# pxl-th/Monodepth2.jl

Hardware: NVIDIA B200
Metric: train frames/s @416x128 R18: view-synthesis loss path (warp + SSIM/L1 loss, fwd+bwd, 4 scales) (higher is better)
Workload: dtype f32

## Files before the change

monodepth2.jl_b200/csrc/md2_common.cuh:

```cuda
#pragma once
#include <cuda_runtime.h>
#include <stdint.h>
#include <string>
#include <stdio.h>

#include "../../include/md2.h"
#include "md2_math.cuh"

namespace md2 {

std::string& last_error_ref();
int set_error(const char* fmt, ...);

struct Workspace {
    void* ptr = nullptr;
    size_t bytes = 0;
};

}

enum { MD2_WS_PARTIAL = 0, MD2_WS_SUMS, MD2_WS_POSE, MD2_WS_STATS, MD2_WS_DISP, MD2_WS_GDISP,
       MD2_WS_MISC, MD2_WS_AUTOMASK, MD2_WS_COUNT };
enum { MD2_WS_BANKS = 1 + MD2_HOST_LANES };

#include <vector>
struct md2_ctx {
    int device;
    int64_t launches;
    int sm_count = 148;
    int bank = 0;
    int64_t ws_gen[MD2_WS_BANKS] = {};
    md2::Workspace ws[MD2_WS_BANKS][MD2_WS_COUNT];
    int prof_on = 0;
    std::vector<cudaEvent_t> prof_ev;
    size_t prof_used = 0;
    void* host[MD2_HOST_LANES] = {};
    void* opt = nullptr;
    void* taps = nullptr;
    void* replay = nullptr;
};

namespace md2 {

void* ws_get(md2_ctx* ctx, int slot, size_t bytes);
int launch_automask(md2_ctx* ctx, int S, const float* const* frames, const int64_t* frame_ns, const float* target, int64_t target_ns,
                    float* out, int W, int H, int C, int N, cudaStream_t st);

struct DeviceGuard {
    int prev = -1;
    cudaError_t err;
    explicit DeviceGuard(int device) {
        err = cudaGetDevice(&prev);
        if (err == cudaSuccess && prev != device) err = cudaSetDevice(device); else if (err == cudaSuccess) prev = -1;
// ... 74 lines not shown
```

monodepth2.jl_b200/csrc/md2_fused.cu:

```cuda
#include <stdarg.h>
#include <string.h>

#include <atomic>

#include "md2_common.cuh"
#include "md2_fused.cuh"
#include "md2_march.cuh"
#include "md2_march2.cuh"

namespace md2 {

void host_path_destroy(md2_ctx* ctx);
void opt_path_destroy(md2_ctx* ctx);
void replay_destroy(md2_ctx* ctx);
void taps_destroy(md2_ctx* ctx);

std::string& last_error_ref() {
    static thread_local std::string e;
    return e;
}
int set_error(const char* fmt, ...) {
    char buf[512];
    va_list ap;
    va_start(ap, fmt);
    vsnprintf(buf, sizeof(buf), fmt, ap);
    va_end(ap);
    last_error_ref() = buf;
    return 1;
}
void* ws_get(md2_ctx* ctx, int slot, size_t bytes) {
    Workspace& w = ctx->ws[ctx->bank][slot];
    if (w.bytes >= bytes && w.ptr) return w.ptr;
    if (w.ptr) {
        cudaDeviceSynchronize();
        cudaFree(w.ptr);
        w.ptr = nullptr; w.bytes = 0;
    }
    size_t want = bytes + bytes / 4 + 256;
    ctx->ws_gen[ctx->bank]++;
    cudaError_t e = cudaMalloc(&w.ptr, want);
    if (e != cudaSuccess) {
        set_error("workspace cudaMalloc(%zu) failed: %s", want, cudaGetErrorString(e));
        w.ptr = nullptr;
        return nullptr;
    }
    w.bytes = want;
    return w.ptr;
}

__global__ void upsample_kernel(const float* __restrict__ in, float* __restrict__ out, int w, int h,
                                int W, int H, int CN) {
    const long long i = (long long)blockIdx.x * blockDim.x + threadIdx.x;
    if (i >= (long long)W * H * CN) return;
    const int x = (int)(i % W), y = (int)((i / W) % H);
    const long long cn = i / ((long long)W * H);
    const float sx = up_scale(w, W), sy = up_scale(h, H);
    int x0, x1, y0, y1; float fx, fy;
    up_taps(x, w, W, x0, x1, fx);
    up_taps(y, h, H, y0, y1, fy);
    const float* b = in + cn * w * h;
    out[i] = bilerp(b[y0 * w + x0], b[y0 * w + x1], b[y1 * w + x0], b[y1 * w + x1], fx, fy);
}

__global__ void upsample_bwd_kernel(const float* __restrict__ gout, float* __restrict__ gin, int w,
                                    int h, int W, int H, int CN) {
// ... 95 lines not shown
        return;
    }
    const bool do_zero = zero_blocks > 0;
    zero_blocks = zero_blocks < 0 ? -zero_blocks : zero_blocks;
    const int zb = blockIdx.x - nblk - 1, s = zb / zero_blocks, sl = zb - s * zero_blocks;
    const int total = C * p.W * p.H;
    const int per = ((total + zero_blocks - 1) / zero_blocks + 3) & ~3;
    const int i0 = sl * per, i1 = min(i0 + per, total);
    {
        const float* src = p.src[s] + (long long)n * p.src_ns[s];
        for (int i = i0 + 32 * (int)threadIdx.x; i < i1; i += 32 * (int)blockDim.x)
            asm volatile("prefetch.global.L2 [%0];" ::"l"(src + i));
        if (threadIdx.x == 0 && i1 > i0) asm volatile("prefetch.global.L2 [%0];" ::"l"(src + (i1 - 1)));
    }
    if (!do_zero || !p.gsrc[s]) return;
    float* g = p.gsrc[s] + (long long)n * p.src_ns[s];
    if ((reinterpret_cast<uintptr_t>(g) & 15) == 0) {
        for (int i = i0 + 4 * (int)threadIdx.x; i + 3 < i1; i += 4 * (int)blockDim.x) *reinterpret_cast<float4*>(g + i) = make_float4(0.f, 0.f, 0.f, 0.f);
        for (int i = i0 + ((i1 - i0) & ~3) + (int)threadIdx.x; i < i1; i += blockDim.x) g[i] = 0.f;
    } else {
        for (int i = i0 + (int)threadIdx.x; i < i1; i += blockDim.x) g[i] = 0.f;
    }
}

template <int C, int LMAX>
__global__ void __launch_bounds__(32 * PREP_WARPS, 3) prep_kernel(const __grid_constant__ FusedParams p, int strips, int chunks,
                                                               int nblk, int do_stats, float* __restrict__ pose_ab,
                                                               float* __restrict__ part, int zero_blocks) {
    const int n = blockIdx.y;
    pdl_trigger();
    if (blockIdx.x == 0 || (int)blockIdx.x > nblk) { prep_pose_or_zero<C>(p, nblk, pose_ab, zero_blocks); return; }
    const int W = p.W, H = p.H, HW = W * H;
    __shared__ float red[PREP_WARPS][3 * LMAX];
    const int lane = threadIdx.x & 31, warp = threadIdx.x >> 5;
    const int w = (blockIdx.x - 1) * PREP_WARPS + warp;
    const bool active = w < strips * chunks;
    const int cy = w / strips, sx = w - cy * strips;
    const int gx = sx * PREP_COLS + lane;
    const int gxc = gx < W ? gx : W - 1;
    const bool own_col = active && lane < PREP_COLS && gx < W;
    const bool has_right = own_col && gx + 1 < W;
    const int Y0 = active ? cy * PREP_ROWS : 0;
    int yo[PREP_ROWS + 1];
#pragma unroll
    for (int r = 0; r <= PREP_ROWS; ++r) yo[r] = min(Y0 + r, H - 1) * W;

// ... 77 lines not shown
            float v0 = 0.f, v1 = 0.f, v2 = 0.f;
#pragma unroll
            for (int r = 0; r <= PREP_ROWS; ++r) {
                if (r < PREP_ROWS) {
                    const float dr = __shfl_down_sync(0xffffffffu, d[r], 1);
                    v0 = fmaf(fabsf(d[r] - dr), wx[r], v0);
                    v2 += (own_col && Y0 + r < H) ? d[r] : 0.f;
                }
                if (r > 0) v1 = fmaf(fabsf(d[r - 1] - d[r]), wy[r], v1);
            }
            v0 = warp_sum(v0); v1 = warp_sum(v1); v2 = warp_sum(v2);
            if (lane == 0) { red[warp][3 * l] = v0; red[warp][3 * l + 1] = v1; red[warp][3 * l + 2] = v2; }
        }
    }
    if (!do_stats) return;
    __syncthreads();
    if ((int)threadIdx.x < 3 * p.L) {
        float s = 0.f;
#pragma unroll
        for (int k = 0; k < PREP_WARPS; ++k) s += red[k][threadIdx.x];
        const int l = threadIdx.x / 3, k = threadIdx.x - 3 * l;
        part[(((long long)l * p.N + n) * nblk + (blockIdx.x - 1)) * 4 + k] = s;
    }
}

__device__ __forceinline__ float warp_reduce_16(float (&v)[16]) {
    const int lane = threadIdx.x & 31;
#pragma unroll
    for (int half = 8; half >= 1; half >>= 1) {
        const bool up = (lane & half) != 0;
#pragma unroll
        for (int i = 0; i < half; ++i) {
            const float send = up ? v[i] : v[i + half];
            const float keep = up ? v[i + half] : v[i];
            v[i] = keep + __shfl_xor_sync(0xffffffffu, send, half);
        }
    }
    return v[0] + __shfl_xor_sync(0xffffffffu, v[0], 16);
}

template <int C, int NLOW>
__global__ void __launch_bounds__(32 * PREP_WARPS, MD2_PREP_MINB) prep_fast_kernel(const __grid_constant__ FusedParams p, int strips, int chunks,
                                                                    int nblk, float* __restrict__ pose_ab,
                                                                    float* __restrict__ part, int zero_blocks) {
    constexpr int NS = NLOW + 1;
    static_assert(3 * NS <= 16, "one transpose-reduce of 16 values");
// ... 82 lines not shown
                if (r < PREP_ROWS && Y0 + r < H && own_col) out[yo[r]] = d[r];
            }
        }
#pragma unroll
        for (int r = 0; r <= PREP_ROWS; ++r) {
            if (r < PREP_ROWS) {
                const float dr = __shfl_down_sync(0xffffffffu, d[r], 1);
                v[3 * l] = fmaf(fabsf(d[r] - dr), wx[r], v[3 * l]);
                v[3 * l + 2] = fmaf(d[r], mcol * rowm[r], v[3 * l + 2]);
            }
            if (r > 0) v[3 * l + 1] = fmaf(fabsf(d[r - 1] - d[r]), wy[r], v[3 * l + 1]);
        }
    }
    const float tot = warp_reduce_16(v);
    if (lane < 16) red[warp][lane] = tot;
    __syncthreads();
    if ((int)threadIdx.x < 3 * NS) {
        float s = 0.f;
#pragma unroll
        for (int k = 0; k < PREP_WARPS; ++k) s += red[k][threadIdx.x];
        const int l = threadIdx.x / 3, k = threadIdx.x - 3 * l;
        part[(((long long)l * p.N + n) * nblk + (blockIdx.x - 1)) * 4 + k] = s;
    }
}

#ifndef MD2_ROLE_SWAP
#define MD2_ROLE_SWAP 1
#endif
template <int C, int S, bool BWD>
struct MarchCfg {
#ifndef MD2_MAXREG_C1
#define MD2_MAXREG_C1 128
#endif
#ifndef MD2_MAXREG_C3
#define MD2_MAXREG_C3 192
#endif
    static constexpr int MAXREG = C == 1 ? MD2_MAXREG_C1 : MD2_MAXREG_C3;
};

template <int C, int S, bool BWD>
__global__ void __maxnreg__((MarchCfg<C, S, BWD>::MAXREG))
march_kernel(const __grid_constant__ FusedParams p, int strips, int chunks, int q_full, int lgroups) {
    extern __shared__ __align__(16) float wsm[];
    using M = March<C, S, BWD>;
    constexpr int NP = M::NPART;
    const int lane = threadIdx.x & 31;
// ... 15 lines not shown
            asm volatile("mov.u32 %0, %%warpid;" : "=r"(wid));
            *swap_flag = MD2_ROLE_SWAP ? (int)((wid >> 2) & 1u) : 0;
        }
        __syncthreads();
        role ^= *swap_flag;
    }
    for (int it = blockIdx.x; it < items; it += gridDim.x) {
        const int z = it / ipi, rem = it - z * ipi;
        int cy, sx, sx_end;
        if (rem < n_full) { cy = rem / strips; sx = rem - cy * strips; sx_end = sx + 1; }
        else { cy = q_full; sx = (rem - n_full) * strips / lgroups; sx_end = (rem - n_full + 1) * strips / lgroups; }
        for (; sx < sx_end; ++sx) {
            float v[32];
            if (role == 0) M::run_forward(p, sx, cy, z, lane, wsm, gslot, v);
            else M::run_backward(p, sx, cy, z, lane, wsm, gslot, v);
            const float tot = warp_reduce_32(v);
            if (role == 0 ? lane < (BWD ? NSTAT : NP) : (lane >= NSTAT && lane < NP))
                p.partial[((long long)z * ipg + cy * strips + sx) * NP + lane] = tot;
            if (BWD) __syncthreads();
        }
    }
}

template <int C, int S, bool AM, bool DBG, bool GRAD>
__global__ void __maxnreg__((March2<C, S, AM, DBG, GRAD>::MAXREG))
march2_kernel(const __grid_constant__ FusedParams p, int strips, int chunks, int q_full, int lgroups) {
    extern __shared__ __align__(16) float wsm[];
    using M = March2<C, S, AM, DBG, GRAD>;
    constexpr int NP = M::NPART;
    const int lane = threadIdx.x;
    pdl_trigger();
    pdl_wait();
    const int ipg = strips * chunks;
    const int n_full = strips * q_full;
    const int ipi = n_full + (chunks > q_full ? lgroups : 0);
    const int items = ipi * p.L * p.N;
    for (int it = blockIdx.x; it < items; it += gridDim.x) {
        const int z = it / ipi, rem = it - z * ipi;
        int cy, sx, sx_end;
        if (rem < n_full) { cy = rem / strips; sx = rem - cy * strips; sx_end = sx + 1; }
        else { cy = q_full; sx = (rem - n_full) * strips / lgroups; sx_end = (rem - n_full + 1) * strips / lgroups; }
        for (; sx < sx_end; ++sx) {
            float v[32];
            M::run(p, sx, cy, z, lane, wsm, v);
            const float tot = warp_reduce_32(v);
            if (GRAD ? (lane == 0 || (lane >= NSTAT && lane < NP)) : lane < NSTAT)
                p.partial[((long long)z * ipg + cy * strips + sx) * NP + lane] = tot;
        }
    }
}

__device__ __forceinline__ double warp_sum_d(double v) {
#pragma unroll
    for (int o = 16; o > 0; o >>= 1) v += __shfl_xor_sync(0xffffffffu, v, o);
    return v;
}

constexpr int FIN_MAXROWS = 64;
constexpr int FIN_THREADS = 128;
#ifndef MD2_FIN_MINB
#define MD2_FIN_MINB 7
#endif
#ifndef MD2_FIN_UNROLL
#define MD2_FIN_UNROLL 16
#endif
constexpr int FIN_UNROLL = MD2_FIN_UNROLL;
#ifndef MD2_FIN_TIMING
#define MD2_FIN_TIMING 0
#endif

__global__ void __launch_bounds__(FIN_THREADS, MD2_FIN_MINB) finish_kernel(const __grid_constant__ FusedParams p, int NP, int ipg, int bwd, int low_rows) {
    extern __shared__ __align__(16) float vrow[];
    const int lane = threadIdx.x & 31, warp = threadIdx.x >> 5;
    pdl_wait();
    const int LN = p.L * p.N;
    int b = blockIdx.x;
    if (b == 0) {
        if (p.mode == 1 || MD2_FIN_TIMING == 4) return;
        constexpr int GL = 4;
        const int sub = threadIdx.x & (GL - 1);
        for (int z0 = 0; z0 < LN; z0 += FIN_THREADS / GL) {
            const int z = z0 + (threadIdx.x / GL);
            float v[4] = {0.f, 0.f, 0.f, 0.f};
            if (z < LN) {
                const float* pp = p.partial + (long long)z * ipg * NP;
                if (p.mode == 0) {
#pragma unroll 4
                    for (int it = sub; it < ipg; it += GL) {
#pragma unroll
                        for (int k = 0; k < 4; ++k) v[k] += __ldcg(pp + (long long)it * NP + k);
                    }
                } else {
#pragma unroll 8
                    for (int it = sub; it < ipg; it += GL) v[0] += __ldcg(pp + (long long)it * NP);
                    const float4* q = reinterpret_cast<const float4*>(p.prep_part) + (long long)z * p.prep_nblk;
#pragma unroll 8
                    for (int it = sub; it < p.prep_nblk; it += GL) {
                        const float4 t = __ldcg(q + it);
                        v[1] += t.x; v[2] += t.y; v[3] += t.z;
                    }
                }
            }
#pragma unroll
            for (int o = GL / 2; o > 0; o >>= 1)
#pragma unroll
                for (int k = 0; k < 4; ++k) v[k] += __shfl_xor_sync(0xffffffffu, v[k], o);
            if (z < LN && sub == 0) {
                float* st = p.stats_out + (long long)z * NSTAT;
#pragma unroll
                for (int k = 0; k < NSTAT; ++k) st[k] = v[k];
                if (p.saved && p.saved != p.stats_out)
#pragma unroll
                    for (int k = 0; k < NSTAT; ++k) p.saved[(long long)z * NSTAT + k] = v[k];
            }
        }
        __syncthreads();
        if (warp == 0 && p.loss) {
            const double P = (double)p.W * p.H;
            const double cx = 1.0 / ((double)(p.W - 1) * p.H * p.N), cy = 1.0 / ((double)p.W * (p.H - 1) * p.N);
            const double rPN = 1.0 / (P * p.N);
            double acc = 0.0;
            for (int z = lane; z < LN; z += 32) {
                const float* st = p.stats_out + (long long)z * NSTAT;
                const double m = p.normalize_disp ? ((double)st[3] / P + 1e-7) : 1.0;
                acc += (double)st[0] * rPN + (double)p.smooth_w[z / p.N] * (cx * st[1] + cy * st[2]) / m;
            }
            acc = warp_sum_d(acc);
            if (lane == 0) *p.loss = (float)(acc * p.loss_scale);
        }
        return;
    }
    b -= 1;
    if (!bwd) return;
    if (b < p.S * p.N) {
        if (MD2_FIN_TIMING == 2) return;
        constexpr int FIN_PR = FIN_THREADS / 3;
        __shared__ double pacc[FIN_PR][12];
        const int s = b / p.N, nn = b % p.N;
        const int q4 = threadIdx.x % 3, j = threadIdx.x / 3;
        if (j < FIN_PR) {
            double a0 = 0.0, a1 = 0.0, a2 = 0.0, a3 = 0.0;
            const int rows = p.L * ipg;
#pragma unroll 4
            for (int r = j; r < rows; r += FIN_PR) {
                const int l = r / ipg, it = r - l * ipg;
                const float4 t = __ldcg(reinterpret_cast<const float4*>(p.partial + (((long long)l * p.N + nn) * ipg + it) * NP + NSTAT + 12 * s) + q4);
                a0 += (double)t.x; a1 += (double)t.y; a2 += (double)t.z; a3 += (double)t.w;
            }
            pacc[j][4 * q4] = a0; pacc[j][4 * q4 + 1] = a1; pacc[j][4 * q4 + 2] = a2; pacc[j][4 * q4 + 3] = a3;
        }
        __syncthreads();
        if (threadIdx.x < 12) {
            double a = 0.0;
#pragma unroll 6
            for (int q = 0; q < FIN_PR; ++q) a += pacc[q][threadIdx.x];
            pacc[0][threadIdx.x] = a;
        }
        __syncthreads();
        if (threadIdx.x == 0 && MD2_FIN_TIMING != 1) finalize_pose(p.pose, s, nn, &pacc[0][0], &pacc[0][0] + 9);
        return;
    }
// ... 212 lines not shown
        if (rem) {
            if (rem < 8 && env <= 0) continue;
            int k = (int)((R + over) / (rem + over));
            if (k < 1) k = 1;
            if (k > strips) k = strips;
            lg = cdiv(strips, k);
            if (env_group >= 1) lg = env_group < strips ? env_group : strips;
        }
        const long long items = base * q + (rem ? (long long)LN * lg : 0);
        const double longest = rem ? fmax(R + over, cdiv(strips, lg) * (rem + over)) : R + over;
        const double total = (double)base * q * (R + over) + (rem ? (double)base * (rem + over) : 0.0);
        const long long per_sm = (items + sms - 1) / sms;
        const double thr = total / ((double)sms * warps);
        const double chain = (double)((per_sm + warps - 1) / warps) * longest;
        const double cost = thr > chain ? thr : chain;
        if (cost < best - 1e-9) { best = cost; best_R = R; group = lg; }
        if (R == 8) break;
    }
    return best_R;
}

struct TapsEntry {
    int W, H, L, dw[MAX_L], dh[MAX_L];
    int wcount[MAX_L] = {};
    float* dev = nullptr;
    uint64_t last_use = 0;
};
struct TapsCache {
    static constexpr int CAP = 8;
    TapsEntry e[CAP];
    int used = 0;
    uint64_t tick = 0;
};
void taps_destroy(md2_ctx* ctx) {
    TapsCache* tc = static_cast<TapsCache*>(ctx->taps);
    if (!tc) return;
    for (int i = 0; i < tc->used; ++i)
        if (tc->e[i].dev) cudaFree(tc->e[i].dev);
    delete tc;
    ctx->taps = nullptr;
}
static int taps_get(md2_ctx* ctx, const md2_vsl_desc* d, FusedParams& p, cudaStream_t st) {
    if (!ctx->taps) ctx->taps = new TapsCache();
    TapsCache* tc = static_cast<TapsCache*>(ctx->taps);
    ++tc->tick;
    TapsEntry* hit = nullptr;
    for (int i = 0; i < tc->used && !hit; ++i) {
        TapsEntry& e = tc->e[i];
        if (e.W == d->W && e.H == d->H && e.L == d->L && memcmp(e.dw, d->disp_w, sizeof(int) * d->L) == 0 && memcmp(e.dh, d->disp_h, sizeof(int) * d->L) == 0) hit = &e;
    }
    const int W = d->W, H = d->H;
    if (!hit) {
        cudaStreamCaptureStatus cs = cudaStreamCaptureStatusNone;
        if (cudaStreamIsCapturing(st, &cs) != cudaSuccess || cs != cudaStreamCaptureStatusNone)
            return set_error("internal: tap tables of a new shape requested under stream capture");
        if (tc->used < TapsCache::CAP) hit = &tc->e[tc->used++];
        else {
            hit = &tc->e[0];
            for (int i = 1; i < tc->used; ++i) if (tc->e[i].last_use < hit->last_use) hit = &tc->e[i];
            MD2_CHECK(cudaDeviceSynchronize());
            cudaFree(hit->dev); hit->dev = nullptr;
            for (int b = 0; b < MD2_WS_BANKS; ++b) ctx->ws_gen[b]++;
        }
        std::vector<float> h;
        for (int l = 0; l < d->L; ++l) {
            if (d->disp_w[l] == W && d->disp_h[l] == H) continue;
            std::vector<int> i0s[2], i1s[2];
            std::vector<float> fs[2];
            for (int pass = 0; pass < 2; ++pass) {
                const int n = pass ? H : W, m = pass ? d->disp_h[l] : d->disp_w[l];
                i0s[pass].resize(n); i1s[pass].resize(n); fs[pass].resize(n);
                for (int x = 0; x < n; ++x) {
                    up_taps(x, m, n, i0s[pass][x], i1s[pass][x], fs[pass][x]);
                    float e[4] = {0.f, 0.f, fs[pass][x], 0.f};
                    memcpy(&e[0], &i0s[pass][x], 4); memcpy(&e[1], &i1s[pass][x], 4);
                    h.insert(h.end(), e, e + 4);
                }
            }
            std::vector<float> wts;
            for (int pass = 0; pass < 2; ++pass) {
                const int n = pass ? H : W, m = pass ? d->disp_h[l] : d->disp_w[l];
                for (int i = 0; i < m; ++i) {
                    auto wgt = [&](int x) { return (i0s[pass][x] == i ? 1.f - fs[pass][x] : 0.f) + (i1s[pass][x] == i ? fs[pass][x] : 0.f); };
                    int lo = 0, hi = n - 1;
                    while (lo < hi && wgt(lo) == 0.f) ++lo;
                    while (hi > lo && wgt(hi) == 0.f) --hi;
                    const int cnt = hi - lo + 1, start = (int)wts.size();
                    for (int x = lo; x <= hi; ++x) wts.push_back(wgt(x));
                    float e[4] = {0.f, 0.f, 0.f, 0.f};
                    memcpy(&e[0], &lo, 4); memcpy(&e[1], &cnt, 4); memcpy(&e[2], &start, 4);
                    h.insert(h.end(), e, e + 4);
                }
            }
            while (wts.size() & 3) wts.push_back(0.f);
            h.insert(h.end(), wts.begin(), wts.end());
            hit->wcount[l] = (int)wts.size();
        }
        MD2_CHECK(cudaMalloc(&hit->dev, sizeof(float) * (h.size() + 4)));
        MD2_CHECK(cudaMemcpy(hit->dev, h.data(), sizeof(float) * h.size(), cudaMemcpyHostToDevice));
        hit->W = W; hit->H = H; hit->L = d->L;
        memset(hit->dw, 0, sizeof(hit->dw)); memset(hit->dh, 0, sizeof(hit->dh));
        memcpy(hit->dw, d->disp_w, sizeof(int) * d->L); memcpy(hit->dh, d->disp_h, sizeof(int) * d->L);
    }
    hit->last_use = tc->tick;
    const float* q = hit->dev;
    for (int l = 0; l < d->L; ++l) {
        if (d->disp_w[l] == W && d->disp_h[l] == H) { p.tap_x[l] = p.tap_y[l] = p.inv_x[l] = p.inv_y[l] = p.inv_w[l] = nullptr; continue; }
        p.tap_x[l] = q; q += (size_t)4 * W;
        p.tap_y[l] = q; q += (size_t)4 * H;
        p.inv_x[l] = q; q += (size_t)4 * d->disp_w[l];
        p.inv_y[l] = q; q += (size_t)4 * d->disp_h[l];
        p.inv_w[l] = q; q += (size_t)hit->wcount[l];
    }
    return 0;
}

static int check_desc(const md2_vsl_desc* d, bool need_loss_inputs) {
    MD2_REQUIRE(d != nullptr, "null descriptor");
    MD2_REQUIRE(d->W >= 2 && d->H >= 2 && d->W <= 65535 && d->H <= 32767, "W, H must be in 2..65535 / 2..32767");
    MD2_REQUIRE((long long)d->W * d->H * d->C < (1LL << 31), "one image must have fewer than 2^31 elements");
    MD2_REQUIRE(d->W <= 12288, "W must be <= 12288 (one image row is staged in shared memory)");
    MD2_REQUIRE(d->N >= 1, "N must be >= 1");
    MD2_REQUIRE(d->C == 1 || d->C == 3, "C must be 1 or 3");
    MD2_REQUIRE(d->S >= 1 && d->S <= MAX_S, "S must be 1 or 2");
    MD2_REQUIRE(d->K && d->invK, "K / invK are null");
    for (int s = 0; s < d->S; ++s) {
        MD2_REQUIRE(d->source[s] != nullptr, "null source image");
        MD2_REQUIRE(d->rot[s] && d->trans[s], "null pose");
    }
    if (need_loss_inputs) {
        MD2_REQUIRE(d->L >= 1 && d->L <= MAX_L, "L must be in 1..8");
        MD2_REQUIRE((long long)d->L * d->N <= 65535, "L*N too large");
        MD2_REQUIRE(d->target != nullptr, "null target image");
        for (int l = 0; l < d->L; ++l) {
            MD2_REQUIRE(d->disparity[l] != nullptr, "null disparity");
// ... 43 lines not shown
        int64_t ns[MAX_S];
        for (int s = 0; s < S; ++s) ns[s] = d->source_image_stride[s];
        if (launch_automask(ctx, S, d->source, ns, d->target, d->target_image_stride, am, W, H, C, N, st)) return 1;
        p.automask = am;
    }
    p.dbg = (bwd && !use_march_v1()) ? d->debug_choices : nullptr;
    if (d->debug_choices) MD2_REQUIRE(p.dbg != nullptr, "debug_choices is served by the value + gradient calls only");
    {
        const float mind = (float)(1.0 / (double)d->max_depth), maxd = (float)(1.0 / (double)d->min_depth);
        p.depth_a = maxd - mind; p.depth_b = mind;
    }
    int n_low = 0, low_rows = 0;
    for (int l = 0; l < L; ++l) {
        p.smooth_w[l] = d->smooth_weight[l];
        p.disp[l] = d->disparity[l]; p.dw[l] = d->disp_w[l]; p.dh[l] = d->disp_h[l];
        p.usx[l] = up_scale(d->disp_w[l], W); p.usy[l] = up_scale(d->disp_h[l], H);
        p.gdisp[l] = bwd ? d->grad_disparity[l] : nullptr;
        if (bwd) MD2_REQUIRE(d->grad_disparity[l] != nullptr, "null grad_disparity");
        if (d->disp_w[l] != W || d->disp_h[l] != H) {
            ++n_low;
            low_rows += d->disp_h[l];
        }
    }
    if (n_low && taps_get(ctx, d, p, st)) return 1;
    {
        const size_t img = (size_t)N * W * H;
        float* dscr = n_low ? (float*)ws_get(ctx, MD2_WS_DISP, sizeof(float) * img * n_low) : nullptr;
        float* gscr = (n_low && bwd) ? (float*)ws_get(ctx, MD2_WS_GDISP, sizeof(float) * img * n_low) : nullptr;
        if (n_low && (!dscr || (bwd && !gscr))) return 1;
        int k = 0;
        for (int l = 0; l < L; ++l) {
            const bool native = d->disp_w[l] == W && d->disp_h[l] == H;
            p.dfull[l] = native ? d->disparity[l] : dscr + img * k;
            p.gfull[l] = !bwd ? nullptr : (native ? d->grad_disparity[l] : gscr + img * k);
            if (!native) ++k;
        }
    }
    p.loss_scale = d->loss_scale;
    p.gloss = gloss;
    p.normalize_disp = d->normalize_disparity;
    p.mode = mode;
    fill_pose_io(d, p.pose);

    const bool v2 = !use_march_v1();
    p.m_R = choose_march_rows(W, H, L * N, v2 || bwd, ctx->sm_count, v2 ? march2_resident_of(C, S, p.automask != nullptr, bwd) : march_resident_of(C, S, bwd), p.m_group);
    static const bool dbg_env = getenv("MD2_DEBUG") != nullptr, generic_env = getenv("MD2_PREP_GENERIC") != nullptr;
    if (dbg_env) fprintf(stderr, "[md2] chunk height %d, %d groups of short last chunks per (scale, image)\n", p.m_R, p.m_group);
    const int tiles = cdiv(W, (v2 || bwd) ? 28 : 30) * cdiv(H, p.m_R);
    const int NP = NSTAT + 12 * S;
    p.pose_slot = 0;
    const int prep_strips = cdiv(W, PREP_COLS), prep_chunks = cdiv(H, PREP_ROWS);
    const int prep_nblk = cdiv((long long)prep_strips * prep_chunks, PREP_WARPS);
    const int do_stats = mode == MODE_FWDBWD;
    const bool zero_gs = bwd && d->zero_grad_source != 0;
    const int aux_blocks = bwd ? max(1, min(64, cdiv((long long)C * W * H, 8192))) : 0;
    const int zero_blocks = zero_gs ? aux_blocks : -aux_blocks;
    float* pose_ab = (float*)ws_get(ctx, MD2_WS_POSE, sizeof(float) * 24 * S * N);
    float* partial = (float*)ws_get(ctx, MD2_WS_PARTIAL, sizeof(float) * (size_t)tiles * L * N * NP);
    float* stats = (float*)ws_get(ctx, MD2_WS_STATS, sizeof(float) * (size_t)L * N * NSTAT);
    float* part2 = (float*)ws_get(ctx, MD2_WS_MISC, sizeof(float) * (size_t)prep_nblk * L * N * 4);
    if (!pose_ab || !partial || !stats || !part2) return 1;
    p.pose_ab = pose_ab; p.pose_e = pose_ab + (size_t)12 * S * N; p.partial = partial;
    p.stats = stats; p.stats_out = stats; p.saved = (mode == MODE_BWD) ? nullptr : d->saved;
    if (mode == MODE_BWD && d->saved) p.stats = d->saved;
    p.loss = (mode == MODE_BWD) ? nullptr : d->loss;
    p.prep_part = do_stats ? part2 : nullptr;
    p.prep_nblk = prep_nblk;

    cudaEvent_t evp0 = nullptr, evp3 = nullptr;
    if (ctx->prof_on == 2) {
        while (ctx->prof_used + 4 > ctx->prof_ev.size()) {
            cudaEvent_t e;
            MD2_CHECK(cudaEventCreate(&e));
            ctx->prof_ev.push_back(e);
        }
        evp0 = ctx->prof_ev[ctx->prof_used + 2]; evp3 = ctx->prof_ev[ctx->prof_used + 3];
        MD2_CHECK(cudaEventRecord(evp0, st));
    }
    {
        const int nb = (do_stats || n_low) ? prep_nblk : 0;
        dim3 g(1 + nb + S * aux_blocks, N);
        bool usual = nb > 0 && L >= 1 && L <= 4 && n_low == L - 1 && d->disp_w[L - 1] == W && d->disp_h[L - 1] == H;
        if (generic_env) usual = false;
#define MD2_PREPF(CC, NL) prep_fast_kernel<CC, NL><<<g, 32 * PREP_WARPS, 0, st>>>(p, prep_strips, prep_chunks, nb, pose_ab, part2, zero_blocks)
#define MD2_PREP(CC, LL) prep_kernel<CC, LL><<<g, 32 * PREP_WARPS, 0, st>>>(p, prep_strips, prep_chunks, nb, do_stats, pose_ab, part2, zero_blocks)
        if (usual && C == 1)      { if (L == 1) MD2_PREPF(1, 0); else if (L == 2) MD2_PREPF(1, 1); else if (L == 3) MD2_PREPF(1, 2); else MD2_PREPF(1, 3); }
        else if (usual)           { if (L == 1) MD2_PREPF(3, 0); else if (L == 2) MD2_PREPF(3, 1); else if (L == 3) MD2_PREPF(3, 2); else MD2_PREPF(3, 3); }
        else if (C == 1) { if (L == 1) MD2_PREP(1, 1); else if (L <= 4) MD2_PREP(1, 4); else MD2_PREP(1, 8); }
        else        { if (L == 1) MD2_PREP(3, 1); else if (L <= 4) MD2_PREP(3, 4); else MD2_PREP(3, 8); }
#undef MD2_PREPF
// ... 3 lines not shown

    cudaEvent_t ev0 = nullptr, ev1 = nullptr;
    if (ctx->prof_on) {
        if (ctx->prof_used + 2 > ctx->prof_ev.size()) {
            for (int k = 0; k < 2; ++k) {
                cudaEvent_t e;
                MD2_CHECK(cudaEventCreate(&e));
                ctx->prof_ev.push_back(e);
            }
        }
        ev0 = ctx->prof_ev[ctx->prof_used]; ev1 = ctx->prof_ev[ctx->prof_used + 1];
        ctx->prof_used += ctx->prof_on == 2 ? 4 : 2;
        MD2_CHECK(cudaEventRecord(ev0, st));
    }
    if (v2) {
        const bool viz = d->viz_loss || d->viz_warped[0] || (S > 1 && d->viz_warped[S - 1]);
        if (!bwd || viz) { if (dispatch_march2(ctx, C, S, p, st, false)) return 1; }
        if (bwd) { if (dispatch_march2(ctx, C, S, p, st, true)) return 1; }
    }
    else if (bwd) { if (dispatch_march<true>(ctx, C, S, p, st)) return 1; }
    else     { if (dispatch_march<false>(ctx, C, S, p, st)) return 1; }
    if (ev1) MD2_CHECK(cudaEventRecord(ev1, st));
    {
        const int blocks = 1 + (bwd ? S * N + low_rows * N : 0);
        MD2_CHECK(launch_after(2, finish_kernel, dim3(blocks), dim3(FIN_THREADS), sizeof(float) * ((W + 3) & ~3), st, p, NP, tiles, bwd ? 1 : 0, low_rows));
        MD2_LAUNCH_CHECK(ctx);
    }
    if (evp3) MD2_CHECK(cudaEventRecord(evp3, st));
    return 0;
}

struct ReplayEntry {
    md2_vsl_desc desc;
    int mode; float seed; int64_t ws_gen;
    uint64_t hash = 0;
    int seen = 0;
    cudaGraphExec_t exec = nullptr;
    int launches = 0;
    uint64_t last_use = 0;
};
struct ReplayCache {
    static constexpr int CAP = 64;
    ReplayEntry e[CAP];
    int used = 0;
    uint64_t tick = 0;
    cudaStream_t cap_stream = nullptr;
};
// ... 247 lines not shown
    return 0;
}

}

extern "C" {

const char* md2_version(void) { return "md2_b200 0.1.0 (sm_100a)"; }
const char* md2_last_error(void) { return md2::last_error_ref().c_str(); }

int md2_create(int device, md2_ctx** out) {
    if (!out) return md2::set_error("md2_create: null out pointer");
    int count = 0;
    cudaError_t e = cudaGetDeviceCount(&count);
    if (e != cudaSuccess || count == 0)
        return md2::set_error("md2_create: no CUDA device (%s); this library has no CPU fallback",
                              cudaGetErrorString(e));
    if (device < 0 || device >= count) return md2::set_error("md2_create: bad device %d", device);
    md2_ctx* c = new md2_ctx();
    c->device = device;
    c->launches = 0;
    c->sm_count = 148;
    cudaDeviceGetAttribute(&c->sm_count, cudaDevAttrMultiProcessorCount, device);
    *out = c;
    return 0;
}

int md2_destroy(md2_ctx* ctx) {
    if (!ctx) return 0;
    md2::DeviceGuard guard(ctx->device);
    cudaDeviceSynchronize();
    for (int b = 0; b < MD2_WS_BANKS; ++b)
        for (int i = 0; i < MD2_WS_COUNT; ++i)
            if (ctx->ws[b][i].ptr) cudaFree(ctx->ws[b][i].ptr);
    for (cudaEvent_t e : ctx->prof_ev) cudaEventDestroy(e);
    md2::host_path_destroy(ctx);
    md2::opt_path_destroy(ctx);
    md2::replay_destroy(ctx);
    md2::taps_destroy(ctx);
    delete ctx;
    return 0;
}

int64_t md2_launch_count(const md2_ctx* ctx) { return ctx ? ctx->launches : 0; }

int md2_profile_enable(md2_ctx* ctx, int32_t on) {
// ... 81 lines not shown
```

monodepth2.jl_b200/csrc/md2_fused.cuh:

```cuda
#pragma once
#include "md2_math.cuh"

namespace md2 {

constexpr int MAX_S = 2;
constexpr int MAX_L = 8;
constexpr int NSTAT = 4;

struct PoseIO {
    int mode;
    const float* rot[MAX_S];
    const float* trans[MAX_S];
    int invert[MAX_S];
    const float* K; const float* invK;
    float* grot[MAX_S];
    float* gtrans[MAX_S];
};

struct FusedParams {
    int W, H, N, L, S;
    const float* tgt; long long tgt_ns;
    const float* src[MAX_S]; long long src_ns[MAX_S];
    float* gsrc[MAX_S];
    const float* disp[MAX_L];
// ... 5 lines not shown
    const float* stats;
    float* partial;
    float depth_a, depth_b;
    float smooth_w[MAX_L];
    float loss_scale;
    float gloss;
    int normalize_disp;
    float* viz_warped[MAX_S];
    float* viz_loss;
    int mode;
    float* stats_out;
    float* saved;
    float* loss;
    PoseIO pose;
    int m_R, m_group, pose_slot;
    const float* dfull[MAX_L];
    float* gfull[MAX_L];
    const float* prep_part;
    int prep_nblk;
    float usx[MAX_L], usy[MAX_L];
    const float* tap_x[MAX_L]; const float* tap_y[MAX_L];
    const float* inv_x[MAX_L]; const float* inv_y[MAX_L]; const float* inv_w[MAX_L];
    int* dbg;
};

#if defined(__CUDA_ARCH__)
#define MD2_ATOMIC_ADD(p, v) atomicAdd((p), (v))
__device__ __forceinline__ float md2_rcp_approx(float x) {
    float r;
    asm("rcp.approx.ftz.f32 %0, %1;" : "=f"(r) : "f"(x));
    return r;
}
#define MD2_RCP_FAST(x) md2_rcp_approx(x)
#define MD2_EXP(x) __expf(x)
#else
#define MD2_ATOMIC_ADD(p, v) (*(p) += (v))
#define MD2_RCP_FAST(x) (1.0f / (x))
#define MD2_EXP(x) expf(x)
#endif

MD2_HD float rcp_acc(float x) {
#if defined(__CUDA_ARCH__)
    const float r = md2_rcp_approx(x);
    return fmaf(r, fmaf(-x, r, 1.0f), r);
#else
    return 1.0f / x;
// ... 184 lines not shown
```

Measured before the change: 106,700.

## Fuse tail reductions and disparity adjoint into prep and march kernels via last-block counters

```diff
diff --git a/monodepth2.jl_b200/csrc/md2_common.cuh b/monodepth2.jl_b200/csrc/md2_common.cuh
--- a/monodepth2.jl_b200/csrc/md2_common.cuh
+++ b/monodepth2.jl_b200/csrc/md2_common.cuh
@@ -20,7 +20,7 @@
 }
 
 enum { MD2_WS_PARTIAL = 0, MD2_WS_SUMS, MD2_WS_POSE, MD2_WS_STATS, MD2_WS_DISP, MD2_WS_GDISP,
-       MD2_WS_MISC, MD2_WS_AUTOMASK, MD2_WS_COUNT };
+       MD2_WS_MISC, MD2_WS_AUTOMASK, MD2_WS_COUNTERS, MD2_WS_GTOT, MD2_WS_COUNT };
 enum { MD2_WS_BANKS = 1 + MD2_HOST_LANES };
 
 #include <vector>
@@ -29,6 +29,7 @@
     int64_t launches;
     int sm_count = 148;
     int bank = 0;
+    int fin_legacy = 0;
     int64_t ws_gen[MD2_WS_BANKS] = {};
     md2::Workspace ws[MD2_WS_BANKS][MD2_WS_COUNT];
     int prof_on = 0;
diff --git a/monodepth2.jl_b200/csrc/md2_fused.cu b/monodepth2.jl_b200/csrc/md2_fused.cu
--- a/monodepth2.jl_b200/csrc/md2_fused.cu
+++ b/monodepth2.jl_b200/csrc/md2_fused.cu
@@ -1,6 +1,7 @@
 #include <stdarg.h>
 #include <string.h>
 
+#include <algorithm>
 #include <atomic>
 
 #include "md2_common.cuh"
@@ -41,6 +42,12 @@
     cudaError_t e = cudaMalloc(&w.ptr, want);
     if (e != cudaSuccess) {
         set_error("workspace cudaMalloc(%zu) failed: %s", want, cudaGetErrorString(e));
+        w.ptr = nullptr;
+        return nullptr;
+    }
+    if (slot == MD2_WS_COUNTERS && (e = cudaMemset(w.ptr, 0, want)) != cudaSuccess) {
+        set_error("workspace cudaMemset failed: %s", cudaGetErrorString(e));
+        cudaFree(w.ptr);
         w.ptr = nullptr;
         return nullptr;
     }
@@ -182,6 +189,36 @@
         for (int i = i0 + (int)threadIdx.x; i < i1; i += blockDim.x) g[i] = 0.f;
     }
 }
+
+__device__ __forceinline__ void prep_finish_image(const FusedParams& p, int nblk, const float* __restrict__ part, int L) {
+    __shared__ int last;
+    const int n = blockIdx.y;
+    __threadfence();
+    __syncthreads();
+    if (threadIdx.x == 0) {
+        last = atomicAdd(p.prep_cnt + n, 1) == nblk - 1;
+        if (last) p.prep_cnt[n] = 0;
+    }
+    __syncthreads();
+    const int lane = threadIdx.x & 31, l = threadIdx.x >> 5;
+    if (!last || l >= L) return;
+    __threadfence();
+    const float4* pp = reinterpret_cast<const float4*>(part) + ((long long)l * p.N + n) * nblk;
+    float a = 0.f, b = 0.f, c = 0.f;
+    for (int k = lane; k < nblk; k += 32) {
+        const float4 q = __ldcg(pp + k);
+        a += q.x; b += q.y; c += q.z;
+    }
+#pragma unroll
+    for (int o = 16; o > 0; o >>= 1) {
+        a += __shfl_xor_sync(0xffffffffu, a, o); b += __shfl_xor_sync(0xffffffffu, b, o); c += __shfl_xor_sync(0xffffffffu, c, o);
+    }
+    if (lane == 0) {
+        float* st = const_cast<float*>(p.stats) + ((long long)l * p.N + n) * NSTAT;
+        st[1] = a; st[2] = b; st[3] = c;
+    }
+}
+static_assert(MAX_L <= PREP_WARPS, "one warp per scale in prep_finish_image");
 
 template <int C, int LMAX>
 __global__ void __launch_bounds__(32 * PREP_WARPS, 3) prep_kernel(const __grid_constant__ FusedParams p, int strips, int chunks,
@@ -305,6 +342,7 @@
         const int l = threadIdx.x / 3, k = threadIdx.x - 3 * l;
         part[(((long long)l * p.N + n) * nblk + (blockIdx.x - 1)) * 4 + k] = s;
     }
+    if (p.prep_cnt) prep_finish_image(p, nblk, part, p.L);
 }
 
 __device__ __forceinline__ float warp_reduce_16(float (&v)[16]) {
@@ -433,6 +471,7 @@
         const int l = threadIdx.x / 3, k = threadIdx.x - 3 * l;
         part[(((long long)l * p.N + n) * nblk + (blockIdx.x - 1)) * 4 + k] = s;
     }
+    if (p.prep_cnt) prep_finish_image(p, nblk, part, NS);
 }
 
 #ifndef MD2_ROLE_SWAP
@@ -494,6 +533,114 @@
     }
 }
 
+template <int NP>
+__device__ __forceinline__ void march2_group_sum(const FusedParams& p, int z, int ipg, int lane) {
+    static_assert(NP % 4 == 0 && NP / 4 <= 8, "one float4 column per lane of a row set");
+    const int q = lane & 7, rs = lane >> 3;
+    double a[4] = {0.0, 0.0, 0.0, 0.0};
+    if (q < NP / 4) {
+        const float4* base = reinterpret_cast<const float4*>(p.partial + (long long)z * ipg * NP) + q;
+#pragma unroll 8
+        for (int r = rs; r < ipg; r += 4) {
+            const float4 t = __ldcg(base + (long long)r * (NP / 4));
+            a[0] += (double)t.x; a[1] += (double)t.y; a[2] += (double)t.z; a[3] += (double)t.w;
+        }
+    }
+#pragma unroll
+    for (int k = 0; k < 4; ++k) {
+        const double t0 = __shfl_sync(0xffffffffu, a[k], q), t1 = __shfl_sync(0xffffffffu, a[k], q + 8);
+        const double t2 = __shfl_sync(0xffffffffu, a[k], q + 16), t3 = __shfl_sync(0xffffffffu, a[k], q + 24);
+        a[k] = ((t0 + t1) + t2) + t3;
+    }
+    if (lane < NP / 4)
+#pragma unroll
+        for (int k = 0; k < 4; ++k) p.gtot[(long long)z * NP + 4 * lane + k] = a[k];
+}
+
+template <int SMEM>
+__device__ __forceinline__ void march2_adjoint_code(const FusedParams& p, int l, int n, int cx, int cc, int strips, int lane, float* wsm) {
+    const int* rng = p.adj_rng[l];
+    const int xa = rng[cx], xb = rng[cx + 1], ya = rng[2 * strips + cc], yb = rng[2 * strips + cc + 1];
+    if (xa >= xb || ya >= yb) return;
+    const float4* ix = reinterpret_cast<const float4*>(p.inv_x[l]);
+    const float4* iy = reinterpret_cast<const float4*>(p.inv_y[l]);
+    const float* __restrict__ wts = p.inv_w[l];
+    const int X0 = __float_as_int(__ldg(ix + xa).x);
+    const float4 el = __ldg(ix + xb - 1);
+    const int ncols = __float_as_int(el.x) + __float_as_int(el.y) - X0;
+    const int W = p.W, w = p.dw[l], h = p.dh[l], nxi = xb - xa;
+    const float* g = p.gfull[l] + (long long)n * W * p.H + X0;
+    float* gd = p.gdisp[l] + (long long)n * h * w;
+    const int rows_per = SMEM / ncols;
+    for (int y0 = ya; y0 < yb; y0 += rows_per) {
+        const int nyi = min(rows_per, yb - y0);
+        for (int j = lane; j < nyi * ncols; j += 32) {
+            const int r = j / ncols, c = j - r * ncols;
+            const float4 e = __ldg(iy + y0 + r);
+            const int ylo = __float_as_int(e.x), ny = __float_as_int(e.y);
+            const float* __restrict__ wy = wts + __float_as_int(e.z);
+            const float* gp = g + (long long)ylo * W + c;
+            float acc = 0.f;
+#pragma unroll 8
+            for (int k = 0; k < ny; ++k) acc = fmaf(__ldg(wy + k), __ldcg(gp + (long long)k * W), acc);
+            wsm[j] = acc;
+        }
+        __syncwarp();
+        for (int j = lane; j < nyi * nxi; j += 32) {
+            const int r = j / nxi, xi = xa + (j - r * nxi);
+            const float4 e = __ldg(ix + xi);
+            const int nx = __float_as_int(e.y);
+            const float* vr = wsm + r * ncols + (__float_as_int(e.x) - X0);
+            const float* __restrict__ wx = wts + __float_as_int(e.z);
+            float acc = 0.f;
+#pragma unroll 4
+            for (int k = 0; k < nx; ++k) acc = fmaf(__ldg(wx + k), vr[k], acc);
+            gd[(long long)(y0 + r) * w + xi] = acc;
+        }
+        __syncwarp();
+    }
+}
+
+__device__ __forceinline__ int march2_segment_count(const FusedParams& p, int sx, int cy, int z, int strips, int chunks, int lane) {
+    const int l = z / p.N, n = z - l * p.N;
+    int* acnt = p.adj_cnt[l];
+    __threadfence();
+    __syncwarp();
+    bool mine = false;
+    if (acnt) {
+        const int ncx = 2 * strips - 1, ncc = 2 * chunks - 1;
+        const int cx = 2 * sx + lane % 3 - 1, cc = 2 * cy + lane / 3 - 1;
+        if (lane < 9 && cx >= 0 && cx < ncx && cc >= 0 && cc < ncc) {
+            const int need = (1 + (cx & 1)) * (1 + (cc & 1));
+            if (need == 1) mine = true;
+            else {
+                int* c = acnt + ((long long)n * ncc + cc) * ncx + cx;
+                if (atomicAdd(c, 1) == need - 1) { *c = 0; mine = true; }
+            }
+        }
+    }
+    if (lane == 9) {
+        mine = atomicAdd(p.grp_cnt + z, 1) == strips * chunks - 1;
+        if (mine) p.grp_cnt[z] = 0;
+    }
+    return (int)__ballot_sync(0xffffffffu, mine);
+}
+
+template <int NP, int SMEM>
+__device__ __forceinline__ void march2_segment_finish(const FusedParams& p, int sx, int cy, int z, int strips, int chunks, int todo,
+                                                      int lane, float* wsm) {
+    const int l = z / p.N, n = z - l * p.N;
+    __threadfence();
+    if (todo & (1 << 9)) march2_group_sum<NP>(p, z, strips * chunks, lane);
+    todo &= (1 << 9) - 1;
+    while (todo) {
+        const int b = __ffs(todo) - 1;
+        todo &= todo - 1;
+        march2_adjoint_code<SMEM>(p, l, n, 2 * sx + b % 3 - 1, 2 * cy + b / 3 - 1, strips, lane, wsm);
+    }
+}
+constexpr int M2_PENDING = 8;
+
 template <int C, int S, bool AM, bool DBG, bool GRAD>
 __global__ void __maxnreg__((March2<C, S, AM, DBG, GRAD>::MAXREG))
 march2_kernel(const __grid_constant__ FusedParams p, int strips, int chunks, int q_full, int lgroups) {
@@ -507,6 +654,8 @@
     const int n_full = strips * q_full;
     const int ipi = n_full + (chunks > q_full ? lgroups : 0);
     const int items = ipi * p.L * p.N;
+    __shared__ int pend[GRAD ? M2_PENDING : 1][3];
+    int npend = 0;
     for (int it = blockIdx.x; it < items; it += gridDim.x) {
         const int z = it / ipi, rem = it - z * ipi;
         int cy, sx, sx_end;
@@ -518,7 +667,19 @@
             const float tot = warp_reduce_32(v);
             if (GRAD ? (lane == 0 || (lane >= NSTAT && lane < NP)) : lane < NSTAT)
                 p.partial[((long long)z * ipg + cy * strips + sx) * NP + lane] = tot;
-        }
+            if (GRAD && p.grp_cnt) {
+                const int todo = march2_segment_count(p, sx, cy, z, strips, chunks, lane);
+                if (todo && npend < M2_PENDING) {
+                    if (lane == 0) { pend[npend][0] = z; pend[npend][1] = sx | cy << 16; pend[npend][2] = todo; }
+                    ++npend;
+                }
+            }
+        }
+    }
+    for (int k = 0; k < npend; ++k) {
+        __syncwarp();
+        const int sc = pend[k][1];
+        march2_segment_finish<NP, M::SMEM_FLOATS>(p, sc & 0xffff, sc >> 16, pend[k][0], strips, chunks, pend[k][2], lane, wsm);
     }
 }
 
@@ -549,41 +710,54 @@
     int b = blockIdx.x;
     if (b == 0) {
         if (p.mode == 1 || MD2_FIN_TIMING == 4) return;
-        constexpr int GL = 4;
-        const int sub = threadIdx.x & (GL - 1);
-        for (int z0 = 0; z0 < LN; z0 += FIN_THREADS / GL) {
-            const int z = z0 + (threadIdx.x / GL);
-            float v[4] = {0.f, 0.f, 0.f, 0.f};
-            if (z < LN) {
-                const float* pp = p.partial + (long long)z * ipg * NP;
-                if (p.mode == 0) {
+        if (p.gtot) {
+            for (int z = threadIdx.x; z < LN; z += FIN_THREADS) {
+                const float* s3 = p.stats + (long long)z * NSTAT;
+                const float v[NSTAT] = {(float)__ldcg(p.gtot + (long long)z * NP), __ldcg(s3 + 1), __ldcg(s3 + 2), __ldcg(s3 + 3)};
+                float* st = p.stats_out + (long long)z * NSTAT;
+#pragma unroll
+                for (int k = 0; k < NSTAT; ++k) st[k] = v[k];
+                if (p.saved && p.saved != p.stats_out)
+#pragma unroll
+                    for (int k = 0; k < NSTAT; ++k) p.saved[(long long)z * NSTAT + k] = v[k];
+            }
+        } else {
+            constexpr int GL = 4;
+            const int sub = threadIdx.x & (GL - 1);
+            for (int z0 = 0; z0 < LN; z0 += FIN_THREADS / GL) {
+                const int z = z0 + (threadIdx.x / GL);
+                float v[4] = {0.f, 0.f, 0.f, 0.f};
+                if (z < LN) {
+                    const float* pp = p.partial + (long long)z * ipg * NP;
+                    if (p.mode == 0) {
 #pragma unroll 4
-                    for (int it = sub; it < ipg; it += GL) {
-#pragma unroll
-                        for (int k = 0; k < 4; ++k) v[k] += __ldcg(pp + (long long)it * NP + k);
-                    }
-                } else {
+                        for (int it = sub; it < ipg; it += GL) {
+#pragma unroll
+                            for (int k = 0; k < 4; ++k) v[k] += __ldcg(pp + (long long)it * NP + k);
+                        }
+                    } else {
 #pragma unroll 8
-                    for (int it = sub; it < ipg; it += GL) v[0] += __ldcg(pp + (long long)it * NP);
-                    const float4* q = reinterpret_cast<const float4*>(p.prep_part) + (long long)z * p.prep_nblk;
+                        for (int it = sub; it < ipg; it += GL) v[0] += __ldcg(pp + (long long)it * NP);
+                        const float4* q = reinterpret_cast<const float4*>(p.prep_part) + (long long)z * p.prep_nblk;
 #pragma unroll 8
-                    for (int it = sub; it < p.prep_nblk; it += GL) {
-                        const float4 t = __ldcg(q + it);
-                        v[1] += t.x; v[2] += t.y; v[3] += t.z;
+                        for (int it = sub; it < p.prep_nblk; it += GL) {
+                            const float4 t = __ldcg(q + it);
+                            v[1] += t.x; v[2] += t.y; v[3] += t.z;
+                        }
                     }
                 }
-            }
-#pragma unroll
-            for (int o = GL / 2; o > 0; o >>= 1)
-#pragma unroll
-                for (int k = 0; k < 4; ++k) v[k] += __shfl_xor_sync(0xffffffffu, v[k], o);
-            if (z < LN && sub == 0) {
-                float* st = p.stats_out + (long long)z * NSTAT;
-#pragma unroll
-                for (int k = 0; k < NSTAT; ++k) st[k] = v[k];
-                if (p.saved && p.saved != p.stats_out)
-#pragma unroll
-                    for (int k = 0; k < NSTAT; ++k) p.saved[(long long)z * NSTAT + k] = v[k];
+#pragma unroll
+                for (int o = GL / 2; o > 0; o >>= 1)
+#pragma unroll
+                    for (int k = 0; k < 4; ++k) v[k] += __shfl_xor_sync(0xffffffffu, v[k], o);
+                if (z < LN && sub == 0) {
+                    float* st = p.stats_out + (long long)z * NSTAT;
+#pragma unroll
+                    for (int k = 0; k < NSTAT; ++k) st[k] = v[k];
+                    if (p.saved && p.saved != p.stats_out)
+#pragma unroll
+                        for (int k = 0; k < NSTAT; ++k) p.saved[(long long)z * NSTAT + k] = v[k];
+                }
             }
         }
         __syncthreads();
@@ -609,6 +783,16 @@
         constexpr int FIN_PR = FIN_THREADS / 3;
         __shared__ double pacc[FIN_PR][12];
         const int s = b / p.N, nn = b % p.N;
+        if (p.gtot) {
+            if (threadIdx.x < 12) {
+                double a = 0.0;
+                for (int l = 0; l < p.L; ++l) a += __ldcg(p.gtot + ((long long)l * p.N + nn) * NP + NSTAT + 12 * s + threadIdx.x);
+                pacc[0][threadIdx.x] = a;
+            }
+            __syncthreads();
+            if (threadIdx.x == 0 && MD2_FIN_TIMING != 1) finalize_pose(p.pose, s, nn, &pacc[0][0], &pacc[0][0] + 9);
+            return;
+        }
         const int q4 = threadIdx.x % 3, j = threadIdx.x / 3;
         if (j < FIN_PR) {
             double a0 = 0.0, a1 = 0.0, a2 = 0.0, a3 = 0.0;
@@ -867,7 +1051,10 @@
 
 struct TapsEntry {
     int W, H, L, dw[MAX_L], dh[MAX_L];
+    int R;
     int wcount[MAX_L] = {};
+    int roff[MAX_L] = {};
+    bool adj_ok = false;
     float* dev = nullptr;
     uint64_t last_use = 0;
 };
@@ -885,14 +1072,15 @@
     delete tc;
     ctx->taps = nullptr;
 }
-static int taps_get(md2_ctx* ctx, const md2_vsl_desc* d, FusedParams& p, cudaStream_t st) {
+constexpr int M2_OW = 28;
+static int taps_get(md2_ctx* ctx, const md2_vsl_desc* d, FusedParams& p, cudaStream_t st, int R, bool& adj_ok) {
     if (!ctx->taps) ctx->taps = new TapsCache();
     TapsCache* tc = static_cast<TapsCache*>(ctx->taps);
     ++tc->tick;
     TapsEntry* hit = nullptr;
     for (int i = 0; i < tc->used && !hit; ++i) {
         TapsEntry& e = tc->e[i];
-        if (e.W == d->W && e.H == d->H && e.L == d->L && memcmp(e.dw, d->disp_w, sizeof(int) * d->L) == 0 && memcmp(e.dh, d->disp_h, sizeof(int) * d->L) == 0) hit = &e;
+        if (e.W == d->W && e.H == d->H && e.L == d->L && e.R == R && memcmp(e.dw, d->disp_w, sizeof(int) * d->L) == 0 && memcmp(e.dh, d->disp_h, sizeof(int) * d->L) == 0) hit = &e;
     }
     const int W = d->W, H = d->H;
     if (!hit) {
@@ -907,6 +1095,8 @@
             cudaFree(hit->dev); hit->dev = nullptr;
             for (int b = 0; b < MD2_WS_BANKS; ++b) ctx->ws_gen[b]++;
         }
+        const int strips = cdiv(W, M2_OW), chunks = cdiv(H, R);
+        hit->adj_ok = true;
         std::vector<float> h;
         for (int l = 0; l < d->L; ++l) {
             if (d->disp_w[l] == W && d->disp_h[l] == H) continue;
@@ -923,6 +1113,7 @@
                 }
             }
             std::vector<float> wts;
+            std::vector<int> los[2], his[2];
             for (int pass = 0; pass < 2; ++pass) {
                 const int n = pass ? H : W, m = pass ? d->disp_h[l] : d->disp_w[l];
                 for (int i = 0; i < m; ++i) {
@@ -930,6 +1121,7 @@
                     int lo = 0, hi = n - 1;
                     while (lo < hi && wgt(lo) == 0.f) ++lo;
                     while (hi > lo && wgt(hi) == 0.f) --hi;
+                    los[pass].push_back(lo); his[pass].push_back(hi);
                     const int cnt = hi - lo + 1, start = (int)wts.size();
                     for (int x = lo; x <= hi; ++x) wts.push_back(wgt(x));
                     float e[4] = {0.f, 0.f, 0.f, 0.f};
@@ -937,25 +1129,40 @@
                     h.insert(h.end(), e, e + 4);
                 }
             }
+            hit->roff[l] = (int)wts.size();
+            for (int pass = 0; pass < 2; ++pass) {
+                const int m = pass ? d->disp_h[l] : d->disp_w[l], seg = pass ? R : M2_OW, ncode = 2 * (pass ? chunks : strips) - 1;
+                std::vector<int> first(ncode + 1, m);
+                int prev = 0;
+                for (int i = m - 1; i >= 0; --i) {
+                    const int a = los[pass][i] / seg, b = his[pass][i] / seg, code = a + b;
+                    if (b - a > 1 || (i < m - 1 && code > prev)) { hit->adj_ok = false; break; }
+                    prev = code;
+                    for (int c = 0; c <= code; ++c) first[c] = i;
+                }
+                for (int c = 0; c <= ncode; ++c) wts.push_back(0.f), memcpy(&wts.back(), &first[c], 4);
+            }
             while (wts.size() & 3) wts.push_back(0.f);
             h.insert(h.end(), wts.begin(), wts.end());
             hit->wcount[l] = (int)wts.size();
         }
         MD2_CHECK(cudaMalloc(&hit->dev, sizeof(float) * (h.size() + 4)));
         MD2_CHECK(cudaMemcpy(hit->dev, h.data(), sizeof(float) * h.size(), cudaMemcpyHostToDevice));
-        hit->W = W; hit->H = H; hit->L = d->L;
+        hit->W = W; hit->H = H; hit->L = d->L; hit->R = R;
         memset(hit->dw, 0, sizeof(hit->dw)); memset(hit->dh, 0, sizeof(hit->dh));
         memcpy(hit->dw, d->disp_w, sizeof(int) * d->L); memcpy(hit->dh, d->disp_h, sizeof(int) * d->L);
     }
     hit->last_use = tc->tick;
+    adj_ok = hit->adj_ok;
     const float* q = hit->dev;
     for (int l = 0; l < d->L; ++l) {
-        if (d->disp_w[l] == W && d->disp_h[l] == H) { p.tap_x[l] = p.tap_y[l] = p.inv_x[l] = p.inv_y[l] = p.inv_w[l] = nullptr; continue; }
+        if (d->disp_w[l] == W && d->disp_h[l] == H) { p.tap_x[l] = p.tap_y[l] = p.inv_x[l] = p.inv_y[l] = p.inv_w[l] = nullptr; p.adj_rng[l] = nullptr; continue; }
         p.tap_x[l] = q; q += (size_t)4 * W;
         p.tap_y[l] = q; q += (size_t)4 * H;
         p.inv_x[l] = q; q += (size_t)4 * d->disp_w[l];
         p.inv_y[l] = q; q += (size_t)4 * d->disp_h[l];
         p.inv_w[l] = q; q += (size_t)hit->wcount[l];
+        p.adj_rng[l] = reinterpret_cast<const int*>(p.inv_w[l] + hit->roff[l]);
     }
     return 0;
 }
@@ -1045,7 +1252,6 @@
             low_rows += d->disp_h[l];
         }
     }
-    if (n_low && taps_get(ctx, d, p, st)) return 1;
     {
         const size_t img = (size_t)N * W * H;
         float* dscr = n_low ? (float*)ws_get(ctx, MD2_WS_DISP, sizeof(float) * img * n_low) : nullptr;
@@ -1069,7 +1275,10 @@
     p.m_R = choose_march_rows(W, H, L * N, v2 || bwd, ctx->sm_count, v2 ? march2_resident_of(C, S, p.automask != nullptr, bwd) : march_resident_of(C, S, bwd), p.m_group);
     static const bool dbg_env = getenv("MD2_DEBUG") != nullptr, generic_env = getenv("MD2_PREP_GENERIC") != nullptr;
     if (dbg_env) fprintf(stderr, "[md2] chunk height %d, %d groups of short last chunks per (scale, image)\n", p.m_R, p.m_group);
-    const int tiles = cdiv(W, (v2 || bwd) ? 28 : 30) * cdiv(H, p.m_R);
+    bool adj_ok = false;
+    if (n_low && taps_get(ctx, d, p, st, p.m_R, adj_ok)) return 1;
+    const int strips = cdiv(W, (v2 || bwd) ? M2_OW : 30), chunks = cdiv(H, p.m_R);
+    const int tiles = strips * chunks;
     const int NP = NSTAT + 12 * S;
     p.pose_slot = 0;
     const int prep_strips = cdiv(W, PREP_COLS), prep_chunks = cdiv(H, PREP_ROWS);
@@ -1089,6 +1298,29 @@
     p.loss = (mode == MODE_BWD) ? nullptr : d->loss;
     p.prep_part = do_stats ? part2 : nullptr;
     p.prep_nblk = prep_nblk;
+    bool fused_red = mode == MODE_FWDBWD && v2 && !ctx->fin_legacy;
+    if (fused_red) {
+        const int q_full = H / p.m_R, lgroups = p.m_group > 0 ? std::min(p.m_group, strips) : 1;
+        const long long items = ((long long)strips * q_full + (chunks > q_full ? lgroups : 0)) * L * N;
+        const bool am = p.automask != nullptr;
+        const int res = !p.dbg ? march2_resident_of(C, S, am, true)
+                               : (C == 1 ? (am ? march2_resident<1, 2, true, true>() : march2_resident<1, 2, false, true>())
+                                         : (am ? march2_resident<3, 2, true, true>() : march2_resident<3, 2, false, true>()));
+        const long long grid = std::min(items, (long long)ctx->sm_count * res);
+        fused_red = (items + grid - 1) / grid * (chunks > q_full ? cdiv(strips, lgroups) : 1) <= M2_PENDING;
+    }
+    const bool adj_march = fused_red && adj_ok;
+    if (fused_red) {
+        const size_t per_low = (size_t)N * (2 * strips - 1) * (2 * chunks - 1);
+        int* cnt = (int*)ws_get(ctx, MD2_WS_COUNTERS, sizeof(int) * ((size_t)N + (size_t)L * N + (adj_march ? per_low * n_low : 0)));
+        double* gtot = (double*)ws_get(ctx, MD2_WS_GTOT, sizeof(double) * (size_t)L * N * NP);
+        if (!cnt || !gtot) return 1;
+        p.prep_cnt = cnt; p.grp_cnt = cnt + N; p.gtot = gtot;
+        p.prep_part = nullptr;
+        int* a = cnt + N + (size_t)L * N;
+        for (int l = 0; l < L && adj_march; ++l)
+            if (d->disp_w[l] != W || d->disp_h[l] != H) { p.adj_cnt[l] = a; a += per_low; }
+    }
 
     cudaEvent_t evp0 = nullptr, evp3 = nullptr;
     if (ctx->prof_on == 2) {
@@ -1138,7 +1370,7 @@
     else     { if (dispatch_march<false>(ctx, C, S, p, st)) return 1; }
     if (ev1) MD2_CHECK(cudaEventRecord(ev1, st));
     {
-        const int blocks = 1 + (bwd ? S * N + low_rows * N : 0);
+        const int blocks = 1 + (bwd ? S * N + (adj_march ? 0 : low_rows * N) : 0);
         MD2_CHECK(launch_after(2, finish_kernel, dim3(blocks), dim3(FIN_THREADS), sizeof(float) * ((W + 3) & ~3), st, p, NP, tiles, bwd ? 1 : 0, low_rows));
         MD2_LAUNCH_CHECK(ctx);
     }
@@ -1432,6 +1664,7 @@
     c->launches = 0;
     c->sm_count = 148;
     cudaDeviceGetAttribute(&c->sm_count, cudaDevAttrMultiProcessorCount, device);
+    { const char* e = getenv("MD2_FIN_LEGACY"); c->fin_legacy = e && atoi(e) != 0; }
     *out = c;
     return 0;
 }
diff --git a/monodepth2.jl_b200/csrc/md2_fused.cuh b/monodepth2.jl_b200/csrc/md2_fused.cuh
--- a/monodepth2.jl_b200/csrc/md2_fused.cuh
+++ b/monodepth2.jl_b200/csrc/md2_fused.cuh
@@ -51,6 +51,9 @@
     const float* tap_x[MAX_L]; const float* tap_y[MAX_L];
     const float* inv_x[MAX_L]; const float* inv_y[MAX_L]; const float* inv_w[MAX_L];
     int* dbg;
+    int* prep_cnt;
+    int* grp_cnt; double* gtot;
+    const int* adj_rng[MAX_L]; int* adj_cnt[MAX_L];
 };
 
 #if defined(__CUDA_ARCH__)
```

New measurement: 71490 (median of 6 runs). 0.67x the previous value.
